# fengranMark/HAConvDR

Hardware: AMD Instinct MI355X
Metric: queries/sec (encode+top-100) over N-passage 768-d corpus; HBM GB/s vs peak (higher is better)
Workload: dtype bf16 MFMA operands with fp32 accumulate / LayerNorm / softmax in the encoder (cosine vs the fp32 reference within 1e-3, measured ~1e-5); search scores and order = the fp32 fmaf chain, bit-exact

## Files before the change

haconvdr_amd/csrc/flat_ip.hip:

```cpp
#include "hac_common.h"

#include <algorithm>
#include <type_traits>
#include <cfloat>
#include <climits>
#include <cmath>
#include <cstdlib>
#include <cstring>
#include <thread>
#include <vector>

namespace hac {

std::string &last_error_slot() {
    static thread_local std::string s;
    return s;
}
int fail(int code, const char *fmt, ...) {
    char buf[512];
    va_list ap;
    va_start(ap, fmt);
    vsnprintf(buf, sizeof buf, fmt, ap);
    va_end(ap);
    last_error_slot() = buf;
// ... 2052 lines not shown
        g.seeded = (size_t)4 * g.GA >= (size_t)SPLIT_K2;
        g.n_pass = scan_passes(G, g.round_groups, g.seeded, g.bounds);
        return g;
    }
    float *delta_of(int64_t off) const { return (float *)ws_delta.p + off; }
    u64 *akeys_of(int64_t off) const { return (u64 *)ws_akeys.p + (size_t)off * SPLIT_K2; }

    int split_begin(SplitCtx &c) {
        const int K2 = SPLIT_K2, C2 = SPLIT_C2;
        const int64_t nq = c.nq;
        hipStream_t st = c.st;
        c.terms = c.level == 0 ? tune.split_terms : 3;
        plan_collect(false);
        HAC_TRY(ensure_half_image(st));
        HAC_TRY(ensure_row_image(st));
        HAC_TRY(upload_segs(st));
        c.G = (u32)((ntotal + GROUP_ROWS - 1) / GROUP_ROWS);
        c.chunk = std::min<int64_t>(nq, SPLIT_CHUNK);
        const int n_qtiles_max = (int)((c.chunk + SH_NQ - 1) / SH_NQ);
        c.lds = c.terms == 3 ? ShCfg<3>::LDS : ShCfg<1>::LDS;
        long Pmax = std::max<long>(1, n_cu);
        HAC_TRY(ws_qsplit.reserve((size_t)n_qtiles_max * SH_NQ * d * 2 * (c.terms == 3 ? 2 : 1)));
        HAC_TRY(ws_delta.reserve((size_t)(nq + SH_NQ) * 4));
        HAC_TRY(ws_cand.reserve((size_t)Pmax * SH_NQ * C2 * 8));
        HAC_TRY(ws_partial.reserve((size_t)std::min<int64_t>(c.chunk, SH_NQ) * Pmax * K2 * 8 * MAX_PASSES));
        HAC_TRY(ws_pcnt.reserve((size_t)c.chunk * 4));
        HAC_TRY(ws_thrglob.reserve(((size_t)n_qtiles_max * SH_NQ + THR_CTL_WORDS) * 4));
        HAC_TRY(ws_akeys.reserve((size_t)nq * K2 * 8));
        HAC_TRY(ws_fail.reserve((size_t)nq * 4));
        HAC_TRY(ws_stat.reserve(16));
        HAC_TRY(ws_thr.reserve((size_t)c.chunk * 4));
        if (((size_t)nq + 8) * 4 > h_fb.cap) HAC_TRY(h_fb.reserve(((size_t)nq + 8) * 8));

        c.a = scan_args(nullptr, 0);
        c.a.pos_base = c.pos_base;
        c.a.k = K2;
        c.a.g_step = 1;
        c.a.thr_glob = thrglob();
        c.a.partial = (u64 *)ws_partial.p;
        c.a.partial_cnt = (u32 *)ws_pcnt.p;
        c.sp.qsplit = (const u32x4 *)ws_qsplit.p;
        c.sp.cand = (u64 *)ws_cand.p;
        c.sp.C2 = C2;
        c.sp.K2 = K2;
        c.sp.thr_is_approx = 1;
        return HAC_OK;
    }
// ... 799 lines not shown
```

haconvdr_amd/csrc/scan_split.inc:

```

typedef _Float16 h16;
typedef _Float16 h16x8 __attribute__((ext_vector_type(8)));
typedef _Float16 h16x4 __attribute__((ext_vector_type(4)));
typedef unsigned int u32x4 __attribute__((ext_vector_type(4)));
typedef float f32x4 __attribute__((ext_vector_type(4)));
typedef const __attribute__((address_space(1))) u32x4 *gu4ptr;

constexpr int SH_NT = 8;
constexpr int SH_NQ = 32 * SH_NT;
constexpr int SH_W = 8;
constexpr int SH_GPR = SH_W / 2;
#ifndef SH_RD1
#define SH_RD1 8
#endif
#ifdef SH_STAMP
#ifndef SH_ST_BX
#define SH_ST_BX 5
#endif
__device__ unsigned long long g_sh_stamps[64];
#endif
template <int TERMS> struct ShCfg {
    static constexpr int STEP_BYTES = TERMS == 3 ? 2048 : 1024;
    static constexpr int CD = TERMS == 3 ? 2 : 1;
    static constexpr int TQ = TERMS == 3 ? 2 : 1;
    static constexpr int STEP_PIECES = SH_NT * TQ * 64;
#ifndef SH_KSL1
#define SH_KSL1 4
#endif
    static constexpr int KSL = TERMS == 3 ? 2 : SH_KSL1;
    static constexpr int SLICE = KSL * STEP_PIECES;
    static constexpr int QS_BYTES = 2 * SLICE * 16;
    static constexpr int RD = TERMS == 3 ? 5 : SH_RD1;
    static constexpr int QDMA = SLICE / (SH_W * 64);
    static constexpr bool SCR_OWN = TERMS == 1;
// ... 56 lines not shown
    for (int o = 32; o > 0; o >>= 1) ss += __shfl_xor(ss, o);
    if ((tid & 63) == 0) red[tid >> 6] = ss;
    __syncthreads();
    if (tid == 0) {
        const int d = 4 * K4;
        const float qn = sqrtf((red[0] + red[1] + red[2]) * 1.0002f);
        const float xn = sqrtf(__uint_as_float(*norm2_max_bits) * 1.0002f);
        float dl = split_err_rel(terms, d) * qn * xn + 1.1920928955078125e-7f * sqrtf((float)d) * (qn + xn) + d * 3.5527136788005009e-15f;
        if (!(qn < 60000.f) || !(xn < 60000.f)) dl = INFINITY;
        delta[qi] = qi < nq ? dl : 0.f;
    }
}

typedef __attribute__((address_space(3))) u32 *lds_u32p;
__device__ __forceinline__ u32 lds_inc_rtn(u32 *p) {
    u32 r;
    const u32 addr = (u32)(uintptr_t)(lds_u32p)p;
    asm volatile("ds_add_rtn_u32 %0, %1, %2\n\ts_waitcnt lgkmcnt(0)" : "=v"(r) : "v"(addr), "v"(1u) : "memory");
    return r;
}
__device__ __forceinline__ void lds_set1(u32 *p) {
    const u32 addr = (u32)(uintptr_t)(lds_u32p)p;
    asm volatile("ds_write_b32 %0, %1" ::"v"(addr), "v"(1u) : "memory");
}

constexpr int q_issues_before(int pos, int rd, int ksl) {
    int c = 0;
    for (int j = 1; j < rd; ++j)
        if ((((pos - j) % ksl) + ksl) % ksl == ksl - 2) ++c;
    return c;
}

template <int N> __device__ __forceinline__ void wait_vmcnt() {
    static_assert(N >= 0 && N < 64, "vmcnt is a 6-bit field");
    __builtin_amdgcn_s_waitcnt(0x0F70 | (N & 15) | ((N >> 4) << 14));
}

#ifndef SH_CORPUS_AUX
#define SH_CORPUS_AUX 0
#endif
#ifndef SH_Q_AUX
#define SH_Q_AUX 0
#endif
template <int TERMS, bool MAXIMA, int QT_ACT = 16>
__global__ __launch_bounds__(SH_W * 64) void scanh_kernel(ScanArgs a, SplitArgs sp) {
    static_assert(QT_ACT == 16 || ((QT_ACT == 8 || QT_ACT == 4) && TERMS == 1), "QT_ACT < 16 is a form of the one-product 16x16x32 scan");
    typedef ShCfg<TERMS> Cfg;
    constexpr int NT = SH_NT, NQ = SH_NQ, W = SH_W, NTHR = SH_W * 64, TQ = Cfg::TQ, RD = Cfg::RD;
    static_assert(Cfg::SCR_OWN || Cfg::SORTERS * 512 * 8 <= Cfg::SLICE * 16, "sort scratch must fit the idle query buffer");
    typedef const __attribute__((address_space(1))) void *gvp;
    typedef __attribute__((address_space(3))) void *lvp;
    extern __shared__ __attribute__((aligned(16))) unsigned char smem[];
    const int tid = threadIdx.x;
    const int lane = tid & 63;
    const int w = __builtin_amdgcn_readfirstlane(tid >> 6);
    const int pr = w >> 1, hf = w & 1;
    const int K4 = a.K4;
    const int NSTEP = K4 / 4;
    const int q0 = blockIdx.y * NQ;
    const int NQr = min(NQ, a.nq - q0);
    const int C2 = sp.C2, K2 = sp.K2;

    u32x4 *qs = reinterpret_cast<u32x4 *>(smem);
    unsigned char *ring = smem + Cfg::QS_BYTES + (size_t)w * RD * Cfg::STEP_BYTES;
    u32 *cnt = reinterpret_cast<u32 *>(smem + Cfg::QS_BYTES + (size_t)W * RD * Cfg::STEP_BYTES);
    float *thr = reinterpret_cast<float *>(cnt + NQ);
    u32 *ovf = reinterpret_cast<u32 *>(thr + NQ);
    u32 *need = ovf + 1;
    SegDesc *lseg = reinterpret_cast<SegDesc *>(ovf + 4);
    u64 *cand = sp.cand + ((size_t)blockIdx.y * gridDim.x + blockIdx.x) * NQ * C2;
    gu4ptr qsrc = (gu4ptr)(sp.qsplit) + (size_t)blockIdx.y * NSTEP * Cfg::STEP_PIECES;

    for (int i = tid; i < NQ; i += NTHR) {
        cnt[i] = 0;
        thr[i] = i < NQr ? (a.thr_init ? a.thr_init[q0 + i] - (sp.thr_is_approx ? 0.f : sp.delta[q0 + i]) : -INFINITY) : __builtin_nanf("");
    }
    if (tid == 0) {
        *ovf = 0;
        *need = 0;
        ovf[2] = 0;
    }
    for (int i = tid; i < Cfg::SLICE; i += NTHR) qs[i] = qsrc[i];
    for (int i = tid; i < a.nseg; i += NTHR) lseg[i] = a.segs[i];
    __syncthreads();
    int seg_cur = 0;
    auto group_base = [&](u32 g) {
        int sg = seg_cur;
        while (sg + 1 < a.nseg && g >= lseg[sg + 1].gstart) ++sg;
        seg_cur = sg;
        if constexpr (TERMS == 3) return as_global(lseg[sg].ptr) + (size_t)(g - lseg[sg].gstart) * K4 * GROUP_ROWS;
        else return as_global(reinterpret_cast<const float4 *>(lseg[sg].himg)) + (size_t)(g - lseg[sg].gstart) * K4 * (GROUP_ROWS / 2);
    };
    const int lane_in_group = TERMS == 3 ? ((lane >> 5) * 64 + 32 * hf + (lane & 31)) : (hf * 64 + lane);
// ... 84 lines not shown
    const int q16_lane = (kg >> 1) * Cfg::STEP_PIECES + (kg & 1) * 32 + m16;

    u32x4 ah, al;
    {
#pragma unroll
        for (int t = 0; t < RD; ++t) dma_step(gp, t, t);
        if constexpr (M16) {
            if (q_issuer) dma_q(1, 1);
        }
        wait_vmcnt<0>();
        __builtin_amdgcn_sched_barrier(0);
        if constexpr (M16) {
#pragma unroll
            for (int rt = 0; rt < 2; ++rt) ac[rt] = *reinterpret_cast<const u32x4 *>(rd16 + rt * 256);
        } else {
            f4 c0, c1;
            read_raw(0, c0, c1);
            convert(c0, c1, ah, al);
        }
        asm volatile("" ::: "memory");
        if constexpr (!LATE) dma_step(gp, RD, 0);
    }
    int rg = 1;
    int par = 0;

#define SH_MFMA(accv, av, bv) \
    accv = __builtin_amdgcn_mfma_f32_32x32x16_f16(__builtin_bit_cast(h16x8, av), __builtin_bit_cast(h16x8, bv), accv, 0, 0, 0)
#define SH_MFMA16(accv, av, bv) \
    accv = __builtin_amdgcn_mfma_f32_16x16x32_f16(__builtin_bit_cast(h16x8, av), __builtin_bit_cast(h16x8, bv), accv, 0, 0, 0)

#ifdef SH_STAMP
    unsigned long long stamps[10] = {0, 0, 0, 0, 0, 0, 0, 0, 0, 0};
#ifdef SH_ST_EPI
#define SH_E(i, rr) if (!MAXIMA && r == (rr)) { \
        const unsigned long long tm_ = __builtin_amdgcn_s_memtime(); \
        const u32 ad_ = (u32)(uintptr_t)(lds_u32p)(smem + Cfg::LDS - 512) + (u32)(w * 64 + (i) * 8); \
        asm volatile("ds_write_b64 %0, %1" ::"v"(ad_), "v"(tm_) : "memory"); }
#else
#define SH_E(i, rr)
#endif
#ifdef SH_ST_ALL
#define SH_T(i) if (((i) == 0 || (i) == 5 || (i) == 8 || (i) == 9) && !MAXIMA && r == SH_ST_R) { \
        const unsigned long long tm_ = __builtin_amdgcn_s_memtime(); \
        const u32 ad_ = (u32)(uintptr_t)(lds_u32p)(smem + Cfg::LDS - 256) + (u32)(w * 32 + ((i) == 0 ? 0 : (i) == 5 ? 8 : (i) == 8 ? 16 : 24)); \
        asm volatile("ds_write_b64 %0, %1" ::"v"(ad_), "v"(tm_) : "memory"); }
#else
#define SH_T(i) if (!MAXIMA && r == SH_ST_R && t >= SH_ST_T && t < SH_ST_T + 4) stamps[i] = __builtin_amdgcn_s_memtime()
#endif
#else
#define SH_E(i, rr)
#define SH_T(i)
#endif
    auto rounds = [&](auto issuer_tag) {
    constexpr int ROLE = decltype(issuer_tag)::value;
    const bool ISSUER = ROLE < 0 ? q_issuer : ROLE == 1;
    for (u32 r = 0; r < nrounds; ++r) {
        const u32 g = a.g_first + item * a.g_step;
        const u32 nitem = item + stride;
        const bool have_next = nitem < a.n_items;
        gf4ptr np = have_next ? uniform(group_base(a.g_first + nitem * a.g_step)) : gp;
        f32x16 acc[NT];
        f32x4 acc16[2][2 * NT];
        if constexpr (!M16) {
#pragma unroll
            for (int n = 0; n < NT; ++n)
#pragma unroll
                for (int e = 0; e < 16; ++e) acc[n][e] = 0.f;
        }

        auto step = [&](const int t, auto pos_tag) {
            constexpr int POS = decltype(pos_tag)::value;
            if constexpr (M16) {
                const u32x4 *qb_cur = qs + par * Cfg::SLICE + q16_lane, *qb_nxt = qs + (par ^ 1) * Cfg::SLICE + q16_lane;
                auto bfrag = [&](int buf, int pp, int qt) {
                    return (buf == par ? qb_cur : qb_nxt)[2 * pp * Cfg::STEP_PIECES + (qt >> 1) * 64 + (qt & 1) * 16];
                };
                constexpr int PP = POS >> 1, ODD = POS & 1;
                constexpr bool LASTP = POS == Cfg::KSL - 1;
                SH_T(POS * 2 + 0);
                if (POS == 0 && t == 0) { SH_E(4, SH_ST_R + 1); }
                if (POS == 1 && t == 1) { SH_E(6, SH_ST_R + 1); }
                asm volatile("" ::: "memory");
                if (POS == 0 && t == 0) {
#pragma unroll
                    for (int i = 0; i < BD; ++i)
                        if (i < QT_ACT) bq[i][0] = bfrag(par, 0, i);
                }
                auto tiles = [&](auto fresh_tag) {
                    constexpr bool FRESH = decltype(fresh_tag)::value;
#pragma unroll
                    for (int i = 0; i < 8; ++i) {
                        const int qt = ODD * 8 + i;
                        const u32x4 bh = bq[i][0];
                        if (qt < QT_ACT) {
                        if constexpr (FRESH) {
                            const f32x4 zero = {0.f, 0.f, 0.f, 0.f};
                            acc16[0][qt] = __builtin_amdgcn_mfma_f32_16x16x32_f16(__builtin_bit_cast(h16x8, ac[0]), __builtin_bit_cast(h16x8, bh), zero, 0, 0, 0);
                            acc16[1][qt] = __builtin_amdgcn_mfma_f32_16x16x32_f16(__builtin_bit_cast(h16x8, ac[1]), __builtin_bit_cast(h16x8, bh), zero, 0, 0, 0);
                        } else {
                            SH_MFMA16(acc16[0][qt], ac[0], bh);
                            SH_MFMA16(acc16[1][qt], ac[1], bh);
                        }
                        }
                        if (!ODD) {
                            if (8 + i < QT_ACT) bq[i][0] = bfrag(par, PP, 8 + i);
                        } else if (i < QT_ACT) {
                            if (!LASTP) bq[i][0] = bfrag(par, PP + 1, i);
                            else if (t + 1 < NSTEP) bq[i][0] = bfrag(par ^ 1, 0, i);
                        }
                        __builtin_amdgcn_sched_barrier(0);
                    }
                };
                if (POS < 2 && t == POS) tiles(std::true_type{});
                else tiles(std::false_type{});
                asm volatile("" ::: "memory");
                SH_T(POS * 2 + 1);
                if (POS == 0 && t == 0) { SH_E(5, SH_ST_R + 1); }
                auto handover = [&]() {
                    asm volatile("" ::: "memory");
                    if (ISSUER) wait_vmcnt<Cfg::CD * Cfg::KSL>();
                    asm volatile("s_waitcnt lgkmcnt(0)" ::: "memory");
                    SH_T(8);
                    __builtin_amdgcn_s_barrier();
                    SH_T(9);
                    __builtin_amdgcn_sched_barrier(0);
                    const int NSL = NSTEP / Cfg::KSL;
                    int sn = t / Cfg::KSL + 2;
                    if (sn >= NSL) sn -= NSL;
                    if (ISSUER) dma_q(sn, par);
                };
                if (ODD) {
                    constexpr int LA = LATE ? 1 : 0;
                    constexpr int QISS = q_issues_before(POS, RD - LA, Cfg::KSL);
                    if constexpr (QFAST) {
                        if (ISSUER) wait_vmcnt<Cfg::CD * (RD - 2 - LA) + QISS * 2 * Cfg::QDMA>();
                        else wait_vmcnt<Cfg::CD * (RD - 2 - LA)>();
                    } else {
                        wait_vmcnt<Cfg::CD * (RD - 2 - LA) + QISS * Cfg::QDMA>();
                    }
                    __builtin_amdgcn_sched_barrier(0);
#pragma unroll
                    for (int rt = 0; rt < 2; ++rt) ac[rt] = *reinterpret_cast<const u32x4 *>(rd16 + rg * 1024 + rt * 256);
                    if constexpr (!LATE) asm volatile("s_waitcnt lgkmcnt(0)" ::: "memory");
                }
                if constexpr (LATE) {
                    const int tn = t + RD, rs = rg == 0 ? RD - 1 : rg - 1;
                    if (tn < NSTEP) dma_step(gp, tn, rs);
                    else dma_step(np, tn - NSTEP, rs);
                    rg = rg == RD - 1 ? 0 : rg + 1;
                } else {
                    const int tn = t + RD + 1;
                    if (tn < NSTEP) dma_step(gp, tn, rg);
                    else dma_step(np, tn - NSTEP, rg);
                    rg = rg == RD - 1 ? 0 : rg + 1;
                }
                if (POS == Cfg::KSL - 2) handover();
                if (LASTP) par ^= 1;
                __builtin_amdgcn_sched_barrier(0);
                return;
            }
            constexpr int OPENERS = POS == 0 ? RD / Cfg::KSL : (POS <= RD ? (RD - POS) / Cfg::KSL + 1 : 0);
            asm volatile("" ::: "memory");
            wait_vmcnt<Cfg::CD * (RD - 1) + OPENERS * Cfg::QDMA>();
            __builtin_amdgcn_sched_barrier(0);
            u32x4 nh, nl;
            const u32x4 *qcur = qs + par * Cfg::SLICE + POS * Cfg::STEP_PIECES + lane;
            if (POS == 0) {
#pragma unroll
                for (int i = 0; i < BD; ++i)
#pragma unroll
                    for (int h = 0; h < TQ; ++h) bq[i][h] = qcur[(i * TQ + h) * 64];
            }
            f4 c0, c1;
            read_raw(rg, c0, c1);
#pragma unroll
            for (int n = 0; n < NT; ++n) {
                const u32x4 bh = bq[n % BD][0];
                if (TERMS == 3) {
                    const u32x4 bl = bq[n % BD][TQ - 1];
// ... 13 lines not shown
            }
            asm volatile("" ::: "memory");
            {
                const int tn = t + RD + 1;
                if (tn < NSTEP) dma_step(gp, tn, rg);
                else dma_step(np, tn - NSTEP, rg);
                rg = rg == RD - 1 ? 0 : rg + 1;
            }
            if (POS == 0) {
                asm volatile("" ::: "memory");
                __builtin_amdgcn_sched_barrier(0);
                const int sn = t / Cfg::KSL + 1;
                dma_q(sn == NSTEP / Cfg::KSL ? 0 : sn, par ^ 1);
            }
            if (POS == Cfg::KSL - 1) {
                wait_vmcnt<Cfg::CD * (Cfg::KSL - 1)>();
                __builtin_amdgcn_s_barrier();
                par ^= 1;
            }
            ah = nh;
            al = nl;
            __builtin_amdgcn_sched_barrier(0);
        };
        for (int t = 0; t < NSTEP; t += Cfg::KSL) {
            step(t, std::integral_constant<int, 0>{});
            step(t + 1, std::integral_constant<int, 1>{});
            if constexpr (Cfg::KSL >= 4) {
                step(t + 2, std::integral_constant<int, 2>{});
                step(t + 3, std::integral_constant<int, 3>{});
            }
            if constexpr (Cfg::KSL == 8) {
                step(t + 4, std::integral_constant<int, 4>{});
                step(t + 5, std::integral_constant<int, 5>{});
                step(t + 6, std::integral_constant<int, 6>{});
                step(t + 7, std::integral_constant<int, 7>{});
            }
        }
        SH_E(0, SH_ST_R);
        gp = np;
        if constexpr (MAXIMA) {
            if (have) {
                const long rem = a.n_rows - (long)g * GROUP_ROWS;
                const int rows_valid = rem < GROUP_ROWS ? (int)rem : GROUP_ROWS;
                const int rb = 32 * hf + 4 * hh;
                const size_t S = (size_t)4 * a.n_items;
                if constexpr (M16) {
#pragma unroll
                    for (int qt = 0; qt < (QT_ACT < 2 * NT ? QT_ACT : 2 * NT); ++qt)
#pragma unroll
                        for (int rt = 0; rt < 2; ++rt) {
                            float m = -INFINITY;
#pragma unroll
                            for (int e = 0; e < 4; ++e)
                                if (32 * hf + 16 * rt + 4 * kg + e < rows_valid) m = fmaxf(m, acc16[rt][qt][e]);
                            m = fmaxf(m, __shfl_xor(m, 16));
                            m = fmaxf(m, __shfl_xor(m, 32));
                            if (kg == 0 && qt * 16 + m16 < NQr) sp.maxima[(size_t)(q0 + qt * 16 + m16) * S + (size_t)item * 4 + hf * 2 + rt] = m;
                        }
                } else {
#pragma unroll
                for (int n = 0; n < NT; ++n) {
                    float m = -INFINITY;
#pragma unroll
                    for (int e = 0; e < 16; ++e)
                        if ((e & 3) + 8 * (e >> 2) + rb < rows_valid) m = fmaxf(m, acc[n][e]);
                    if (n * 32 + jl < NQr) sp.maxima[(size_t)(q0 + n * 32 + jl) * S + (size_t)item * 4 + hf * 2 + hh] = m;
                }
                }
            }
            item = nitem;
            have = have_next;
            continue;
        }
#if SH_NOEPI == 1
#pragma unroll
        for (int rt = 0; rt < 2; ++rt)
            asm volatile("" ::"v"(acc16[rt][0]), "v"(acc16[rt][1]), "v"(acc16[rt][2]), "v"(acc16[rt][3]), "v"(acc16[rt][4]), "v"(acc16[rt][5]), "v"(acc16[rt][6]), "v"(acc16[rt][7]),
                         "v"(acc16[rt][8]), "v"(acc16[rt][9]), "v"(acc16[rt][10]), "v"(acc16[rt][11]), "v"(acc16[rt][12]), "v"(acc16[rt][13]), "v"(acc16[rt][14]), "v"(acc16[rt][15]));
        item = nitem;
        have = have_next;
        continue;
#endif
        constexpr bool STAGED = M16 && Cfg::SCR_OWN;
        constexpr int REGION = Cfg::SORTERS * 4096 / SH_W;
#ifdef SH_REC_CAP
        constexpr int REC_CAP = SH_REC_CAP;
#else
        constexpr int REC_CAP = REGION / 48 < 64 ? REGION / 48 : 64;
#endif
        static_assert(!STAGED || (REGION % 16 == 0 && REC_CAP * 48 <= REGION && REC_CAP <= 64), "staging region");
        unsigned char *stg = smem + Cfg::LDS_BASE + (size_t)w * REGION;
        const u32 stg_a = (u32)(uintptr_t)(lds_u32p)stg;
        f32x4 rec0 = {0.f, 0.f, 0.f, 0.f}, rec1 = {0.f, 0.f, 0.f, 0.f};
        u32 rcode = 0u, rfull = 0u;
        u64 *scr = reinterpret_cast<u64 *>(Cfg::SCR_OWN ? smem + Cfg::LDS_BASE : smem + (size_t)(par ^ 1) * Cfg::SLICE * 16) + (size_t)(w % Cfg::SORTERS) * C2;

        constexpr int NTL = M16 ? (QT_ACT < 2 * NT ? QT_ACT : 2 * NT) : NT, NE = M16 ? 8 : 16;
        constexpr int PB = 32 / NE, PMASK = (1 << NE) - 1;
        u32 pw[NTL / PB];
#pragma unroll
        for (int i = 0; i < NTL / PB; ++i) pw[i] = 0u;
        auto pget = [&](int n) { return (pw[n / PB] >> ((n % PB) * NE)) & (u32)PMASK; };
        const int rbase = 32 * hf + 4 * hh;
        auto qof = [&](int tl) { return M16 ? tl * 16 + m16 : tl * 32 + jl; };
        u32 qlc = (u32)(M16 ? m16 : jl) * (u32)C2;
        asm volatile("" : "+v"(qlc));
        auto rof = [&](int x) { return M16 ? 32 * hf + 16 * (x >> 2) + 4 * kg + (x & 3) : (x & 3) + 8 * (x >> 2) + rbase; };
        auto vof = [&](int tl, int x) -> float {
            if constexpr (M16) return acc16[x >> 2][tl][x & 3];
            else return acc[tl][x];
        };
        auto append_record = [&](u32 m) -> u32 {
            const int pl = (int)(rcode & 63u), pn = (int)(rcode >> 8);
            const int pj = pn * 16 + (pl & 15);
            u32 full = 0u;
            while (__any(m != 0u)) {
                if (m != 0u) {
                    const int e = __builtin_ctz(m);
                    m &= m - 1u;
                    float sc = rec0[0];
#pragma unroll
                    for (int x = 1; x < 8; ++x) sc = e == x ? (x < 4 ? rec0[x & 3] : rec1[x & 3]) : sc;
                    const u32 pos = lds_inc_rtn(&cnt[pj]);
                    if (pos < (u32)C2) {
                        const int row = 32 * hf + 16 * (e >> 2) + 4 * (pl >> 4) + (e & 3);
                        cand[(u32)pj * (u32)C2 + pos] = make_key(sc, a.pos_base + g * GROUP_ROWS + row);
                        if (pos >= hw) lds_set1(need);
                    } else {
                        lds_set1(ovf);
                        full |= 1u << e;
                    }
                }
            }
            return full;
        };
        bool direct = false;
        {
            const long rem = a.n_rows - (long)g * GROUP_ROWS;
            const int rows_valid = rem < GROUP_ROWS ? (int)rem : GROUP_ROWS;
            float thn[NTL];
#pragma unroll
            for (int n = 0; n < NTL; ++n) thn[n] = thr[qof(n)];
            asm volatile("s_waitcnt lgkmcnt(0)" ::: "memory");
            if constexpr (STAGED) {
                int base = 0;
                if (have) {
#pragma unroll
                    for (int n = 0; n < NTL; ++n) {
                        const float th = thn[n];
                        float mx;
                        asm("v_max3_f32 %0, %1, %2, %3" : "=v"(mx) : "v"(vof(n, 0)), "v"(vof(n, 1)), "v"(vof(n, 2)));
                        asm("v_max3_f32 %0, %1, %2, %3" : "=v"(mx) : "v"(mx), "v"(vof(n, 3)), "v"(vof(n, 4)));
                        asm("v_max3_f32 %0, %1, %2, %3" : "=v"(mx) : "v"(mx), "v"(vof(n, 5)), "v"(vof(n, 6)));
                        asm("v_max_f32 %0, %1, %2" : "=v"(mx) : "v"(mx), "v"(vof(n, 7)));
                        const unsigned long long bal = __ballot(mx >= th);
                        const int nf = __builtin_popcountll(bal);
                        if (nf == 0) continue;
                        if (base + nf > REC_CAP) {
                            direct = true;
#pragma unroll
                            for (int e = 0; e < NE; ++e) {
                                if (vof(n, e) >= th && rof(e) < rows_valid) pw[n / PB] |= (1u << (e + (n % PB) * NE));
                            }
                        } else {
                            const u32 rank = __builtin_amdgcn_mbcnt_hi((u32)(bal >> 32), __builtin_amdgcn_mbcnt_lo((u32)bal, 0u));
                            const u32 ad = stg_a + __umul24((u32)base + rank, 48u);
                            const u32 code = (u32)(n << 8) | (u32)lane;
                            unsigned long long sv;
                            asm volatile("s_and_saveexec_b64 %0, %1\n\tds_write_b128 %2, %3\n\tds_write_b128 %2, %4 offset:16\n\t"
                                         "ds_write2_b32 %2, %5, %6 offset0:8 offset1:9\n\ts_mov_b64 exec, %0"
                                         : "=&s"(sv)
                                         : "s"(bal), "v"(ad), "v"(acc16[0][n]), "v"(acc16[1][n]), "v"(code), "v"(th)
                                         : "memory", "scc");
                            base += nf;
                        }
                    }
                }
                if (base > 0) {
                    u32 m = 0u;
                    if (lane < base) {
                        const unsigned char *rp = stg + lane * 48;
                        rec0 = *reinterpret_cast<const f32x4 *>(rp);
                        rec1 = *reinterpret_cast<const f32x4 *>(rp + 16);
                        rcode = *reinterpret_cast<const u32 *>(rp + 32);
                        const float rth = *reinterpret_cast<const float *>(rp + 36);
#pragma unroll
                        for (int e = 0; e < 4; ++e) {
                            m |= rec0[e] >= rth ? (1u << e) : 0u;
                            m |= rec1[e] >= rth ? (16u << e) : 0u;
                        }
                        if (rows_valid != GROUP_ROWS) {
#pragma unroll
                            for (int e = 0; e < 8; ++e)
                                if (32 * hf + 16 * (e >> 2) + 4 * (int)((rcode & 63u) >> 4) + (e & 3) >= rows_valid) m &= ~(1u << e);
                        }
                    }
                    rfull = append_record(m);
                }
            } else {
#pragma unroll
            for (int n = 0; n < NTL; ++n) {
                const float th = thn[n];
                if (have) {
                    float mx;
                    if constexpr (NE == 8) {
                        asm("v_max3_f32 %0, %1, %2, %3" : "=v"(mx) : "v"(vof(n, 0)), "v"(vof(n, 1)), "v"(vof(n, 2)));
                        asm("v_max3_f32 %0, %1, %2, %3" : "=v"(mx) : "v"(mx), "v"(vof(n, 3)), "v"(vof(n, 4)));
                        asm("v_max3_f32 %0, %1, %2, %3" : "=v"(mx) : "v"(mx), "v"(vof(n, 5)), "v"(vof(n, 6)));
                        asm("v_max_f32 %0, %1, %2" : "=v"(mx) : "v"(mx), "v"(vof(n, 7)));
                    } else {
                        mx = vof(n, 0);
#pragma unroll
                        for (int e = 1; e < NE; ++e) mx = fmaxf(mx, vof(n, e));
                    }
#if SH_NOEPI == 3
                    asm volatile("" ::"v"(mx));
                    if (false) {
#else
                    if (__any(mx >= th)) {
#endif
#pragma unroll
                        for (int e = 0; e < NE; ++e) {
// ... 1 lines not shown
                            if (v >= th && (rows_valid == GROUP_ROWS || rof(e) < rows_valid)) {
#if SH_NOEPI == 2
                                asm volatile("" ::"v"(v));
                                continue;
#endif
                                const u32 pos = lds_inc_rtn(&cnt[qof(n)]);
                                if (pos < (u32)C2) {
                                    cand[(u32)(n * (M16 ? 16 : 32) * C2) + qlc + pos] = make_key(v, a.pos_base + g * GROUP_ROWS + rof(e));
                                    if (pos >= hw) lds_set1(need);
                                } else {
                                    lds_set1(ovf);
                                    pw[n / PB] |= (1u << (e + (n % PB) * NE));
                                }
                            }
                        }
                    }
                }
            }
            }
        }
        SH_E(1, SH_ST_R);
        for (int pass = 0;; ++pass) {
            bool anyp = false;
            if (pass > 0 || direct) {
#pragma unroll
                for (int i = 0; i < NTL / PB; ++i) anyp |= (pw[i] != 0u);
            }
            if ((pass > 0 || direct) && __any(anyp)) {
#pragma unroll
                for (int n = 0; n < NTL; ++n) {
                    if (pget(n) != 0u) {
                        float sc[NE];
#pragma unroll
                        for (int e = 0; e < NE; ++e) sc[e] = vof(n, e);
                        const int j = qof(n);
                        u32 m = pget(n);
                        while (m) {
                            const int e = __builtin_ctz(m);
                            m &= m - 1u;
                            const u32 pos = lds_inc_rtn(&cnt[j]);
                            if (pos < (u32)C2) {
                                const int row = rof(e);
                                cand[(u32)(n * (M16 ? 16 : 32) * C2) + qlc + pos] = make_key(sc[e], a.pos_base + g * GROUP_ROWS + row);
                                pw[n / PB] &= ~(1u << (e + (n % PB) * NE));
                                if (pos >= hw) lds_set1(need);
                            } else {
                                lds_set1(ovf);
                            }
                        }
                    }
                }
            }
            if constexpr (STAGED) {
                if (pass > 0 && __any(rfull != 0u)) rfull = append_record(rfull);
            }
            if (pass == 0) {
                SH_E(2, SH_ST_R);
                __builtin_amdgcn_s_waitcnt(0xC07F);
                __builtin_amdgcn_s_barrier();
                SH_E(3, SH_ST_R);
                if ((*(volatile u32 *)ovf | *(volatile u32 *)need) == 0u) break;
            }
            __syncthreads();
            const bool over = (*ovf != 0u);
            for (int jj = w; jj < NQr && w < Cfg::SORTERS; jj += Cfg::SORTERS) {
                u32 n = cnt[jj];
                if (n > (u32)C2) n = (u32)C2;
                float t_new = -INFINITY;
                const bool compact = n > hw;
                if (compact) {
                    u64 *cj = cand + (size_t)jj * C2;
                    for (u32 i = lane; i < n; i += 64) scr[i] = cj[i];
                    lds_fence();
                    wave_sort_desc(scr, n, lane);
                    t_new = ord2f((u32)(scr[K2 - 1] >> 32));
                    for (u32 i = lane; i < (u32)K2; i += 64) cj[i] = scr[i];
                }
                if (lane == 0) {
// ... 5 lines not shown
                            atomicMax(&a.thr_glob[q0 + jj], f2ord(t_new));
                        }
                    }
                    const u32 go = __hip_atomic_load(&a.thr_glob[q0 + jj], __ATOMIC_RELAXED, __HIP_MEMORY_SCOPE_AGENT);
                    if (go != 0u) t_cur = fmaxf(t_cur, ord2f(go));
                    thr[jj] = t_cur;
                }
            }
            __syncthreads();
            if (tid == 0) {
                *ovf = 0u;
                *need = 0u;
                ovf[2] = over ? ovf[2] + 1u : 0u;
            }
            if (!over) break;
#pragma unroll
            for (int n = 0; n < NTL; ++n) {
                if (pget(n) == 0u) continue;
                const float th = thr[qof(n)];
#pragma unroll
                for (int e = 0; e < NE; ++e)
                    if ((pw[n / PB] & (1u << (e + (n % PB) * NE))) && !(vof(n, e) >= th)) pw[n / PB] &= ~(1u << (e + (n % PB) * NE));
            }
            if constexpr (STAGED) {
                if (rfull != 0u) {
                    const float th = thr[(int)(rcode >> 8) * 16 + (int)(rcode & 15u)];
#pragma unroll
                    for (int e = 0; e < 8; ++e)
                        if ((rfull & (1u << e)) && !((e < 4 ? rec0[e & 3] : rec1[e & 3]) >= th)) rfull &= ~(1u << e);
                }
            }
            __syncthreads();
            if (__builtin_expect(*(volatile u32 *)(ovf + 2) >= scan_pass_bound(a, SH_GPR * 64 + 4), 0)) {
                static_assert(NQ <= NTHR, "one thread per query of the tile");
                scan_overrun(a, q0, NQr, tid);
                __syncthreads();
                if (tid == 0) ovf[2] = 0u;
                break;
            }
        }
        item = nitem;
        have = have_next;
    }
    };
    if constexpr (QFAST && !MAXIMA) {
        if (w < 4) rounds(std::integral_constant<int, 1>{});
        else rounds(std::integral_constant<int, 0>{});
    } else if constexpr (QFAST) {
        rounds(std::integral_constant<int, -1>{});
    } else {
        rounds(std::integral_constant<int, 1>{});
    }
#undef SH_MFMA

    wait_vmcnt<0>();
#ifdef SH_STAMP
    if (!MAXIMA) {
        __syncthreads();
        for (int i = tid; i < NQ; i += NTHR) atomicAdd(&g_sh_stamps[60], (unsigned long long)min(cnt[i], (u32)C2));
    }
    if (!MAXIMA && blockIdx.x == SH_ST_BX && blockIdx.y == 0 && lane == 0) {
#ifdef SH_ST_EPI
        for (int i = 0; i < 7; ++i) g_sh_stamps[w * 8 + i] = reinterpret_cast<const unsigned long long *>(smem + Cfg::LDS - 512)[w * 8 + i];
#elif defined(SH_ST_ALL)
        for (int i = 0; i < 4; ++i) g_sh_stamps[w * 4 + i] = reinterpret_cast<const unsigned long long *>(smem + Cfg::LDS - 256)[w * 4 + i];
// ... 254 lines not shown
```

Baseline: 8268.

## Weave previous group's threshold filtering into next group's MFMA steps

In the M16 staged path, the per-group epilogue (max-reduce, ballot, staging survivors to LDS, appending candidates) is deferred and interleaved with the next group's MFMA tiles. The previous group's accumulators are kept live, filtered tile by tile during the first steps, and survivors that overflow the LDS staging area are parked in a new per-wave global spill region appended to the candidate workspace. The goal is to hide the epilogue's latency and barrier behind matrix work. In exchange it adds register pressure from the duplicated accumulators, extra global spill traffic, and considerably more complex control flow.

```diff
diff --git a/haconvdr_amd/csrc/flat_ip.hip b/haconvdr_amd/csrc/flat_ip.hip
--- a/haconvdr_amd/csrc/flat_ip.hip
+++ b/haconvdr_amd/csrc/flat_ip.hip
@@ -2098,7 +2098,7 @@
         long Pmax = std::max<long>(1, n_cu);
         HAC_TRY(ws_qsplit.reserve((size_t)n_qtiles_max * SH_NQ * d * 2 * (c.terms == 3 ? 2 : 1)));
         HAC_TRY(ws_delta.reserve((size_t)(nq + SH_NQ) * 4));
-        HAC_TRY(ws_cand.reserve((size_t)Pmax * SH_NQ * C2 * 8));
+        HAC_TRY(ws_cand.reserve((size_t)Pmax * ((size_t)SH_NQ * C2 + SH_SPILL_U64) * 8));
         HAC_TRY(ws_partial.reserve((size_t)std::min<int64_t>(c.chunk, SH_NQ) * Pmax * K2 * 8 * MAX_PASSES));
         HAC_TRY(ws_pcnt.reserve((size_t)c.chunk * 4));
         HAC_TRY(ws_thrglob.reserve(((size_t)n_qtiles_max * SH_NQ + THR_CTL_WORDS) * 4));
diff --git a/haconvdr_amd/csrc/scan_split.inc b/haconvdr_amd/csrc/scan_split.inc
--- a/haconvdr_amd/csrc/scan_split.inc
+++ b/haconvdr_amd/csrc/scan_split.inc
@@ -10,6 +10,9 @@
 constexpr int SH_NQ = 32 * SH_NT;
 constexpr int SH_W = 8;
 constexpr int SH_GPR = SH_W / 2;
+constexpr int SH_SPILL_REC = 2 * SH_NT * 64;
+constexpr size_t SH_SPILL_U64 = (size_t)SH_W * SH_SPILL_REC * 6;
+constexpr u32 SH_REC_FRESH = 0x80000000u;
 #ifndef SH_RD1
 #define SH_RD1 8
 #endif
@@ -112,6 +115,10 @@
 __device__ __forceinline__ void lds_set1(u32 *p) {
     const u32 addr = (u32)(uintptr_t)(lds_u32p)p;
     asm volatile("ds_write_b32 %0, %1" ::"v"(addr), "v"(1u) : "memory");
+}
+__device__ __forceinline__ void lds_set1_w(u32 *p) {
+    const u32 addr = (u32)(uintptr_t)(lds_u32p)p;
+    asm volatile("ds_write_b32 %0, %1\n\ts_waitcnt lgkmcnt(0)" ::"v"(addr), "v"(1u) : "memory");
 }
 
 constexpr int q_issues_before(int pos, int rd, int ksl) {
@@ -158,7 +165,7 @@
     u32 *ovf = reinterpret_cast<u32 *>(thr + NQ);
     u32 *need = ovf + 1;
     SegDesc *lseg = reinterpret_cast<SegDesc *>(ovf + 4);
-    u64 *cand = sp.cand + ((size_t)blockIdx.y * gridDim.x + blockIdx.x) * NQ * C2;
+    u64 *cand = sp.cand + ((size_t)blockIdx.y * gridDim.x + blockIdx.x) * ((size_t)NQ * C2 + SH_SPILL_U64);
     gu4ptr qsrc = (gu4ptr)(sp.qsplit) + (size_t)blockIdx.y * NSTEP * Cfg::STEP_PIECES;
 
     for (int i = tid; i < NQ; i += NTHR) {
@@ -289,6 +296,9 @@
         if constexpr (!LATE) dma_step(gp, RD, 0);
     }
     int rg = 1;
+    u32 fp_g = 0;
+    bool fp_have = false;
+    int brec = 0;
     int par = 0;
 
 #define SH_MFMA(accv, av, bv) \
@@ -321,13 +331,230 @@
     auto rounds = [&](auto issuer_tag) {
     constexpr int ROLE = decltype(issuer_tag)::value;
     const bool ISSUER = ROLE < 0 ? q_issuer : ROLE == 1;
+    constexpr bool WEAVE = M16 && Cfg::SCR_OWN && !MAXIMA && SH_NOEPI != 1;
+    constexpr int NTL16 = QT_ACT < 2 * NT ? QT_ACT : 2 * NT;
+    constexpr int WREGION = Cfg::SORTERS * 4096 / SH_W;
+#ifdef SH_REC_CAP
+    constexpr int WREC_CAP = SH_REC_CAP;
+#else
+    constexpr int WREC_CAP = WREGION / 48 < 64 ? WREGION / 48 : 64;
+#endif
+    static_assert(!WEAVE || (WREGION % 16 == 0 && WREC_CAP * 48 <= WREGION && WREC_CAP <= 64 && Cfg::KSL >= 4), "staging region; filter steps before the first hand-over");
+    f32x4 acc16_w[2][2 * NT];
+    auto fp_rows_valid = [&](const u32 fg) __attribute__((always_inline)) {
+        const long rem = a.n_rows - (long)fg * GROUP_ROWS;
+        return rem < GROUP_ROWS ? (int)rem : GROUP_ROWS;
+    };
+    auto spill_of = [&]() __attribute__((always_inline)) { return reinterpret_cast<u32x4 *>(cand + (size_t)NQ * C2) + (size_t)w * SH_SPILL_REC * 3; };
+    auto append_rec = [&](u32 m, const f32x4 &r0, const f32x4 &r1, const u32 code, const u32 fg) __attribute__((always_inline)) -> u32 {
+        const int pl = (int)(code & 63u), pn = (int)(code >> 8);
+        const int pj = pn * 16 + (pl & 15);
+        u32 full = 0u;
+        while (__any(m != 0u)) {
+            if (m != 0u) {
+                const int e = __builtin_ctz(m);
+                m &= m - 1u;
+                float sc = r0[0];
+#pragma unroll
+                for (int x = 1; x < 8; ++x) sc = e == x ? (x < 4 ? r0[x & 3] : r1[x & 3]) : sc;
+                const u32 pos = lds_inc_rtn(&cnt[pj]);
+                if (pos < (u32)C2) {
+                    const int row = 32 * hf + 16 * (e >> 2) + 4 * (pl >> 4) + (e & 3);
+                    cand[(u32)pj * (u32)C2 + pos] = make_key(sc, a.pos_base + fg * GROUP_ROWS + row);
+                    if (pos >= hw) lds_set1_w(need);
+                } else {
+                    lds_set1_w(ovf);
+                    full |= 1u << e;
+                }
+            }
+        }
+        return full;
+    };
+    auto park = [&, spill_of](const int n, const float th, const unsigned long long bal, const int st, const u32 fg) __attribute__((always_inline)) -> int {
+        const int nrec = st & 255, ngl = st >> 8;
+        const int nf = __builtin_popcountll(bal);
+        const u32 rank = __builtin_amdgcn_mbcnt_hi((u32)(bal >> 32), __builtin_amdgcn_mbcnt_lo((u32)bal, 0u));
+        u32 ln = (u32)lane;
+        asm volatile("" : "+v"(ln));
+        const u32 code = (u32)(n << 8) | ln;
+        if (nrec + nf <= WREC_CAP) {
+            const u32 ad = (u32)(uintptr_t)(lds_u32p)(smem + Cfg::LDS_BASE + (size_t)w * WREGION) + __umul24((u32)nrec + rank, 48u);
+            unsigned long long sv;
+            asm volatile("s_and_saveexec_b64 %0, %1\n\tds_write_b128 %2, %3\n\tds_write_b128 %2, %4 offset:16\n\t"
+                         "ds_write2_b32 %2, %5, %6 offset0:8 offset1:9\n\ts_mov_b64 exec, %0\n\ts_waitcnt lgkmcnt(0)"
+                         : "=&s"(sv)
+                         : "s"(bal), "v"(ad), "v"(acc16_w[0][n]), "v"(acc16_w[1][n]), "v"(code), "v"(th)
+                         : "memory", "scc");
+            return st + nf;
+        } else {
+            if ((bal >> ln) & 1ull) {
+                u32x4 *rp = spill_of() + (size_t)((u32)ngl + rank) * 3;
+                rp[0] = __builtin_bit_cast(u32x4, acc16_w[0][n]);
+                rp[1] = __builtin_bit_cast(u32x4, acc16_w[1][n]);
+                const u32x4 c = {code, __float_as_uint(th), SH_REC_FRESH, 0u};
+                rp[2] = c;
+            }
+            return st + 256 * nf;
+        }
+    };
+    auto filt_tile = [&, park](const int n, const float th, const int st, const u32 fg) __attribute__((always_inline)) -> int {
+        float mx;
+        asm("v_max3_f32 %0, %1, %2, %3" : "=v"(mx) : "v"(acc16_w[0][n][0]), "v"(acc16_w[0][n][1]), "v"(acc16_w[0][n][2]));
+        asm("v_max3_f32 %0, %1, %2, %3" : "=v"(mx) : "v"(mx), "v"(acc16_w[0][n][3]), "v"(acc16_w[1][n][0]));
+        asm("v_max3_f32 %0, %1, %2, %3" : "=v"(mx) : "v"(mx), "v"(acc16_w[1][n][1]), "v"(acc16_w[1][n][2]));
+        asm("v_max_f32 %0, %1, %2" : "=v"(mx) : "v"(mx), "v"(acc16_w[1][n][3]));
+        const unsigned long long bal = __ballot(mx >= th);
+        if (bal != 0ull) return park(n, th, bal, st, fg);
+        return st;
+    };
+    auto records = [&, append_rec, spill_of, fp_rows_valid](const bool retry, const int st, const u32 fg) __attribute__((always_inline)) -> int {
+        u32x4 *spill = spill_of();
+        const int nrec = st & 255, ngl0 = st >> 8;
+        int ngl = ngl0;
+        if (ngl0 > 0) __builtin_amdgcn_fence(__ATOMIC_SEQ_CST, "workgroup");
+        for (int b0 = 0; b0 < ngl0; b0 += 64) {
+            const int i = b0 + lane;
+            u32 m = 0u, om = 0u, code = 0u;
+            f32x4 r0 = {0.f, 0.f, 0.f, 0.f}, r1 = {0.f, 0.f, 0.f, 0.f};
+            if (i < ngl0) {
+                const u32x4 c = spill[(size_t)i * 3 + 2];
+                om = m = c[2];
+                if (m != 0u) {
+                    r0 = __builtin_bit_cast(f32x4, spill[(size_t)i * 3]);
+                    r1 = __builtin_bit_cast(f32x4, spill[(size_t)i * 3 + 1]);
+                    code = c[0];
+                    if (m == SH_REC_FRESH) {
+                        const float rth = __uint_as_float(c[1]);
+                        m = 0u;
+#pragma unroll
+                        for (int e = 0; e < 4; ++e) {
+                            m |= r0[e] >= rth ? (1u << e) : 0u;
+                            m |= r1[e] >= rth ? (16u << e) : 0u;
+                        }
+                        const int rows_valid = fp_rows_valid(fg);
+                        if (rows_valid != GROUP_ROWS) {
+#pragma unroll
+                            for (int e = 0; e < 8; ++e)
+                                if (32 * hf + 16 * (e >> 2) + 4 * (int)((code & 63u) >> 4) + (e & 3) >= rows_valid) m &= ~(1u << e);
+                        }
+                    }
+                    if (retry) {
+                        const float th = thr[(int)(code >> 8) * 16 + (int)(code & 15u)];
+#pragma unroll
+                        for (int e = 0; e < 8; ++e)
+                            if (!((e < 4 ? r0[e & 3] : r1[e & 3]) >= th)) m &= ~(1u << e);
+                    }
+                }
+            }
+            if (!__any(om != 0u)) continue;
+            const u32 full = append_rec(m, r0, r1, code, fg);
+            if (om != full) reinterpret_cast<u32 *>(spill + (size_t)i * 3 + 2)[2] = full;
+        }
+        if (!retry && nrec > 0) {
+            u32 m = 0u, code = 0u;
+            float rth = 0.f;
+            f32x4 r0 = {0.f, 0.f, 0.f, 0.f}, r1 = {0.f, 0.f, 0.f, 0.f};
+            if (lane < nrec) {
+                const unsigned char *rp = smem + Cfg::LDS_BASE + (size_t)w * WREGION + lane * 48;
+                r0 = *reinterpret_cast<const f32x4 *>(rp);
+                r1 = *reinterpret_cast<const f32x4 *>(rp + 16);
+                code = *reinterpret_cast<const u32 *>(rp + 32);
+                rth = *reinterpret_cast<const float *>(rp + 36);
+#pragma unroll
+                for (int e = 0; e < 4; ++e) {
+                    m |= r0[e] >= rth ? (1u << e) : 0u;
+                    m |= r1[e] >= rth ? (16u << e) : 0u;
+                }
+                const int rows_valid = fp_rows_valid(fg);
+                if (rows_valid != GROUP_ROWS) {
+#pragma unroll
+                    for (int e = 0; e < 8; ++e)
+                        if (32 * hf + 16 * (e >> 2) + 4 * (int)((code & 63u) >> 4) + (e & 3) >= rows_valid) m &= ~(1u << e);
+                }
+            }
+            const u32 full = append_rec(m, r0, r1, code, fg);
+            const unsigned long long fb = __ballot(full != 0u);
+            if (fb != 0ull) {
+                const u32 rank = __builtin_amdgcn_mbcnt_hi((u32)(fb >> 32), __builtin_amdgcn_mbcnt_lo((u32)fb, 0u));
+                if (full != 0u) {
+                    u32x4 *rp = spill + (size_t)((u32)ngl + rank) * 3;
+                    rp[0] = __builtin_bit_cast(u32x4, r0);
+                    rp[1] = __builtin_bit_cast(u32x4, r1);
+                    const u32x4 c = {code, __float_as_uint(rth), full, 0u};
+                    rp[2] = c;
+                }
+                ngl += __builtin_popcountll(fb);
+            }
+        }
+        return 256 * ngl;
+    };
+    auto compact_lists = [&, records](int st, const u32 fg) __attribute__((always_inline)) {
+        u64 *scr = reinterpret_cast<u64 *>(smem + Cfg::LDS_BASE) + (size_t)(w % Cfg::SORTERS) * C2;
+        for (;;) {
+            __syncthreads();
+            const bool over = (*ovf != 0u);
+            for (int jj = w; jj < NQr && w < Cfg::SORTERS; jj += Cfg::SORTERS) {
+                u32 n = cnt[jj];
+                if (n > (u32)C2) n = (u32)C2;
+                float t_new = -INFINITY;
+                const bool compact = n > hw;
+                if (compact) {
+                    u64 *cj = cand + (size_t)jj * C2;
+                    for (u32 i = lane; i < n; i += 64) scr[i] = cj[i];
+                    lds_fence();
+                    wave_sort_desc(scr, n, lane);
+                    t_new = ord2f((u32)(scr[K2 - 1] >> 32));
+                    for (u32 i = lane; i < (u32)K2; i += 64) cj[i] = scr[i];
+                }
+                if (lane == 0) {
+                    float t_cur = thr[jj];
+                    if (compact) {
+                        cnt[jj] = K2;
+                        if (t_new > t_cur) {
+                            t_cur = t_new;
+                            atomicMax(&a.thr_glob[q0 + jj], f2ord(t_new));
+                        }
+                    }
+                    const u32 go = __hip_atomic_load(&a.thr_glob[q0 + jj], __ATOMIC_RELAXED, __HIP_MEMORY_SCOPE_AGENT);
+                    if (go != 0u) t_cur = fmaxf(t_cur, ord2f(go));
+                    thr[jj] = t_cur;
+                }
+            }
+            __syncthreads();
+            if (tid == 0) {
+                *ovf = 0u;
+                *need = 0u;
+                ovf[2] = over ? ovf[2] + 1u : 0u;
+            }
+            if (!over) break;
+            __syncthreads();
+            if (__builtin_expect(*(volatile u32 *)(ovf + 2) >= scan_pass_bound(a, SH_GPR * 64 + 4), 0)) {
+                static_assert(NQ <= NTHR, "one thread per query of the tile");
+                scan_overrun(a, q0, NQr, tid);
+                __syncthreads();
+                if (tid == 0) ovf[2] = 0u;
+                break;
+            }
+            st = records(true, st, fg);
+        }
+    };
+    if constexpr (WEAVE) {
+#pragma unroll
+        for (int rt = 0; rt < 2; ++rt)
+#pragma unroll
+            for (int qt = 0; qt < 2 * NT; ++qt) acc16_w[rt][qt] = f32x4{0.f, 0.f, 0.f, 0.f};
+#pragma unroll
+        for (int i = 0; i < BD; ++i)
+            if (i < QT_ACT) bq[i][0] = (qs + par * Cfg::SLICE + q16_lane)[(i >> 1) * 64 + (i & 1) * 16];
+    }
     for (u32 r = 0; r < nrounds; ++r) {
         const u32 g = a.g_first + item * a.g_step;
         const u32 nitem = item + stride;
         const bool have_next = nitem < a.n_items;
-        gf4ptr np = have_next ? uniform(group_base(a.g_first + nitem * a.g_step)) : gp;
+        gf4ptr np = !WEAVE && have_next ? uniform(group_base(a.g_first + nitem * a.g_step)) : gp;
         f32x16 acc[NT];
-        f32x4 acc16[2][2 * NT];
+        f32x4 acc16_r[2][2 * NT];
+        auto &acc16 = *(WEAVE ? &acc16_w : &acc16_r);
         if constexpr (!M16) {
 #pragma unroll
             for (int n = 0; n < NT; ++n)
@@ -335,8 +562,10 @@
                 for (int e = 0; e < 16; ++e) acc[n][e] = 0.f;
         }
 
-        auto step = [&](const int t, auto pos_tag) {
+        auto step = [&, filt_tile, records, compact_lists](const int t, auto pos_tag, auto first_tag) {
             constexpr int POS = decltype(pos_tag)::value;
+            constexpr bool FIRST = decltype(first_tag)::value;
+            (void)filt_tile, (void)records, (void)compact_lists;
             if constexpr (M16) {
                 const u32x4 *qb_cur = qs + par * Cfg::SLICE + q16_lane, *qb_nxt = qs + (par ^ 1) * Cfg::SLICE + q16_lane;
                 auto bfrag = [&](int buf, int pp, int qt) {
@@ -348,18 +577,28 @@
                 if (POS == 0 && t == 0) { SH_E(4, SH_ST_R + 1); }
                 if (POS == 1 && t == 1) { SH_E(6, SH_ST_R + 1); }
                 asm volatile("" ::: "memory");
-                if (POS == 0 && t == 0) {
+                if (FIRST && POS == 0 && !WEAVE) {
 #pragma unroll
                     for (int i = 0; i < BD; ++i)
                         if (i < QT_ACT) bq[i][0] = bfrag(par, 0, i);
                 }
-                auto tiles = [&](auto fresh_tag) {
-                    constexpr bool FRESH = decltype(fresh_tag)::value;
+                auto tiles = [&, filt_tile](auto fresh_tag, auto filt_tag) {
+                    constexpr bool FRESH = decltype(fresh_tag)::value, FILT = decltype(filt_tag)::value;
+                    float thc = 0.f;
+                    if constexpr (FILT) {
+                        if (ODD * 8 < QT_ACT) thc = thr[ODD * 8 * 16 + m16];
+                    }
 #pragma unroll
                     for (int i = 0; i < 8; ++i) {
                         const int qt = ODD * 8 + i;
                         const u32x4 bh = bq[i][0];
                         if (qt < QT_ACT) {
+                        if constexpr (FILT) {
+                            float thn = 0.f;
+                            if (i + 1 < 8 && qt + 1 < QT_ACT) thn = thr[(qt + 1) * 16 + m16];
+                            brec = filt_tile(qt, fp_have ? thc : __builtin_nanf(""), brec, fp_g);
+                            thc = thn;
+                        }
                         if constexpr (FRESH) {
                             const f32x4 zero = {0.f, 0.f, 0.f, 0.f};
                             acc16[0][qt] = __builtin_amdgcn_mfma_f32_16x16x32_f16(__builtin_bit_cast(h16x8, ac[0]), __builtin_bit_cast(h16x8, bh), zero, 0, 0, 0);
@@ -373,13 +612,21 @@
                             if (8 + i < QT_ACT) bq[i][0] = bfrag(par, PP, 8 + i);
                         } else if (i < QT_ACT) {
                             if (!LASTP) bq[i][0] = bfrag(par, PP + 1, i);
-                            else if (t + 1 < NSTEP) bq[i][0] = bfrag(par ^ 1, 0, i);
+                            else if (WEAVE || t + 1 < NSTEP) bq[i][0] = bfrag(par ^ 1, 0, i);
                         }
                         __builtin_amdgcn_sched_barrier(0);
                     }
                 };
-                if (POS < 2 && t == POS) tiles(std::true_type{});
-                else tiles(std::false_type{});
+                u32 flags = 0u;
+                if constexpr (WEAVE && FIRST && LASTP) flags = *(volatile u32 *)ovf | *(volatile u32 *)need;
+                if constexpr (FIRST && POS < 2) {
+                    tiles(std::true_type{}, std::integral_constant<bool, WEAVE>{});
+                    if constexpr (WEAVE && POS == 1) {
+                        if (brec != 0) brec = records(false, brec, fp_g);
+                    }
+                } else {
+                    tiles(std::false_type{}, std::false_type{});
+                }
                 asm volatile("" ::: "memory");
                 SH_T(POS * 2 + 1);
                 if (POS == 0 && t == 0) { SH_E(5, SH_ST_R + 1); }
@@ -422,6 +669,16 @@
                     rg = rg == RD - 1 ? 0 : rg + 1;
                 }
                 if (POS == Cfg::KSL - 2) handover();
+                if constexpr (WEAVE && FIRST && LASTP) {
+                    if (flags != 0u) {
+                        compact_lists(brec, fp_g);
+#pragma unroll
+                        for (int i = 0; i < BD; ++i)
+                            if (i < QT_ACT) bq[i][0] = bfrag(par ^ 1, 0, i);
+                    }
+                    brec = 0;
+                    if (have_next) np = uniform(group_base(a.g_first + nitem * a.g_step));
+                }
                 if (LASTP) par ^= 1;
                 __builtin_amdgcn_sched_barrier(0);
                 return;
@@ -481,19 +738,25 @@
             al = nl;
             __builtin_amdgcn_sched_barrier(0);
         };
-        for (int t = 0; t < NSTEP; t += Cfg::KSL) {
-            step(t, std::integral_constant<int, 0>{});
-            step(t + 1, std::integral_constant<int, 1>{});
+        auto slice = [&](const int t, auto first_tag) {
+            step(t, std::integral_constant<int, 0>{}, first_tag);
+            step(t + 1, std::integral_constant<int, 1>{}, first_tag);
             if constexpr (Cfg::KSL >= 4) {
-                step(t + 2, std::integral_constant<int, 2>{});
-                step(t + 3, std::integral_constant<int, 3>{});
+                step(t + 2, std::integral_constant<int, 2>{}, first_tag);
+                step(t + 3, std::integral_constant<int, 3>{}, first_tag);
             }
             if constexpr (Cfg::KSL == 8) {
-                step(t + 4, std::integral_constant<int, 4>{});
-                step(t + 5, std::integral_constant<int, 5>{});
-                step(t + 6, std::integral_constant<int, 6>{});
-                step(t + 7, std::integral_constant<int, 7>{});
-            }
+                step(t + 4, std::integral_constant<int, 4>{}, first_tag);
+                step(t + 5, std::integral_constant<int, 5>{}, first_tag);
+                step(t + 6, std::integral_constant<int, 6>{}, first_tag);
+                step(t + 7, std::integral_constant<int, 7>{}, first_tag);
+            }
+        };
+        if constexpr (M16) {
+            slice(0, std::true_type{});
+            for (int t = Cfg::KSL; t < NSTEP; t += Cfg::KSL) slice(t, std::false_type{});
+        } else {
+            for (int t = 0; t < NSTEP; t += Cfg::KSL) slice(t, std::false_type{});
         }
         SH_E(0, SH_ST_R);
         gp = np;
@@ -531,6 +794,13 @@
             have = have_next;
             continue;
         }
+        if constexpr (WEAVE) {
+            fp_g = g;
+            fp_have = have;
+            item = nitem;
+            have = have_next;
+            continue;
+        }
 #if SH_NOEPI == 1
 #pragma unroll
         for (int rt = 0; rt < 2; ++rt)
@@ -540,18 +810,6 @@
         have = have_next;
         continue;
 #endif
-        constexpr bool STAGED = M16 && Cfg::SCR_OWN;
-        constexpr int REGION = Cfg::SORTERS * 4096 / SH_W;
-#ifdef SH_REC_CAP
-        constexpr int REC_CAP = SH_REC_CAP;
-#else
-        constexpr int REC_CAP = REGION / 48 < 64 ? REGION / 48 : 64;
-#endif
-        static_assert(!STAGED || (REGION % 16 == 0 && REC_CAP * 48 <= REGION && REC_CAP <= 64), "staging region");
-        unsigned char *stg = smem + Cfg::LDS_BASE + (size_t)w * REGION;
-        const u32 stg_a = (u32)(uintptr_t)(lds_u32p)stg;
-        f32x4 rec0 = {0.f, 0.f, 0.f, 0.f}, rec1 = {0.f, 0.f, 0.f, 0.f};
-        u32 rcode = 0u, rfull = 0u;
         u64 *scr = reinterpret_cast<u64 *>(Cfg::SCR_OWN ? smem + Cfg::LDS_BASE : smem + (size_t)(par ^ 1) * Cfg::SLICE * 16) + (size_t)(w % Cfg::SORTERS) * C2;
 
         constexpr int NTL = M16 ? (QT_ACT < 2 * NT ? QT_ACT : 2 * NT) : NT, NE = M16 ? 8 : 16;
@@ -569,31 +827,6 @@
             if constexpr (M16) return acc16[x >> 2][tl][x & 3];
             else return acc[tl][x];
         };
-        auto append_record = [&](u32 m) -> u32 {
-            const int pl = (int)(rcode & 63u), pn = (int)(rcode >> 8);
-            const int pj = pn * 16 + (pl & 15);
-            u32 full = 0u;
-            while (__any(m != 0u)) {
-                if (m != 0u) {
-                    const int e = __builtin_ctz(m);
-                    m &= m - 1u;
-                    float sc = rec0[0];
-#pragma unroll
-                    for (int x = 1; x < 8; ++x) sc = e == x ? (x < 4 ? rec0[x & 3] : rec1[x & 3]) : sc;
-                    const u32 pos = lds_inc_rtn(&cnt[pj]);
-                    if (pos < (u32)C2) {
-                        const int row = 32 * hf + 16 * (e >> 2) + 4 * (pl >> 4) + (e & 3);
-                        cand[(u32)pj * (u32)C2 + pos] = make_key(sc, a.pos_base + g * GROUP_ROWS + row);
-                        if (pos >= hw) lds_set1(need);
-                    } else {
-                        lds_set1(ovf);
-                        full |= 1u << e;
-                    }
-                }
-            }
-            return full;
-        };
-        bool direct = false;
         {
             const long rem = a.n_rows - (long)g * GROUP_ROWS;
             const int rows_valid = rem < GROUP_ROWS ? (int)rem : GROUP_ROWS;
@@ -601,62 +834,7 @@
 #pragma unroll
             for (int n = 0; n < NTL; ++n) thn[n] = thr[qof(n)];
             asm volatile("s_waitcnt lgkmcnt(0)" ::: "memory");
-            if constexpr (STAGED) {
-                int base = 0;
-                if (have) {
-#pragma unroll
-                    for (int n = 0; n < NTL; ++n) {
-                        const float th = thn[n];
-                        float mx;
-                        asm("v_max3_f32 %0, %1, %2, %3" : "=v"(mx) : "v"(vof(n, 0)), "v"(vof(n, 1)), "v"(vof(n, 2)));
-                        asm("v_max3_f32 %0, %1, %2, %3" : "=v"(mx) : "v"(mx), "v"(vof(n, 3)), "v"(vof(n, 4)));
-                        asm("v_max3_f32 %0, %1, %2, %3" : "=v"(mx) : "v"(mx), "v"(vof(n, 5)), "v"(vof(n, 6)));
-                        asm("v_max_f32 %0, %1, %2" : "=v"(mx) : "v"(mx), "v"(vof(n, 7)));
-                        const unsigned long long bal = __ballot(mx >= th);
-                        const int nf = __builtin_popcountll(bal);
-                        if (nf == 0) continue;
-                        if (base + nf > REC_CAP) {
-                            direct = true;
-#pragma unroll
-                            for (int e = 0; e < NE; ++e) {
-                                if (vof(n, e) >= th && rof(e) < rows_valid) pw[n / PB] |= (1u << (e + (n % PB) * NE));
-                            }
-                        } else {
-                            const u32 rank = __builtin_amdgcn_mbcnt_hi((u32)(bal >> 32), __builtin_amdgcn_mbcnt_lo((u32)bal, 0u));
-                            const u32 ad = stg_a + __umul24((u32)base + rank, 48u);
-                            const u32 code = (u32)(n << 8) | (u32)lane;
-                            unsigned long long sv;
-                            asm volatile("s_and_saveexec_b64 %0, %1\n\tds_write_b128 %2, %3\n\tds_write_b128 %2, %4 offset:16\n\t"
-                                         "ds_write2_b32 %2, %5, %6 offset0:8 offset1:9\n\ts_mov_b64 exec, %0"
-                                         : "=&s"(sv)
-                                         : "s"(bal), "v"(ad), "v"(acc16[0][n]), "v"(acc16[1][n]), "v"(code), "v"(th)
-                                         : "memory", "scc");
-                            base += nf;
-                        }
-                    }
-                }
-                if (base > 0) {
-                    u32 m = 0u;
-                    if (lane < base) {
-                        const unsigned char *rp = stg + lane * 48;
-                        rec0 = *reinterpret_cast<const f32x4 *>(rp);
-                        rec1 = *reinterpret_cast<const f32x4 *>(rp + 16);
-                        rcode = *reinterpret_cast<const u32 *>(rp + 32);
-                        const float rth = *reinterpret_cast<const float *>(rp + 36);
-#pragma unroll
-                        for (int e = 0; e < 4; ++e) {
-                            m |= rec0[e] >= rth ? (1u << e) : 0u;
-                            m |= rec1[e] >= rth ? (16u << e) : 0u;
-                        }
-                        if (rows_valid != GROUP_ROWS) {
-#pragma unroll
-                            for (int e = 0; e < 8; ++e)
-                                if (32 * hf + 16 * (e >> 2) + 4 * (int)((rcode & 63u) >> 4) + (e & 3) >= rows_valid) m &= ~(1u << e);
-                        }
-                    }
-                    rfull = append_record(m);
-                }
-            } else {
+            {
 #pragma unroll
             for (int n = 0; n < NTL; ++n) {
                 const float th = thn[n];
@@ -704,11 +882,11 @@
         SH_E(1, SH_ST_R);
         for (int pass = 0;; ++pass) {
             bool anyp = false;
-            if (pass > 0 || direct) {
+            if (pass > 0) {
 #pragma unroll
                 for (int i = 0; i < NTL / PB; ++i) anyp |= (pw[i] != 0u);
             }
-            if ((pass > 0 || direct) && __any(anyp)) {
+            if (pass > 0 && __any(anyp)) {
 #pragma unroll
                 for (int n = 0; n < NTL; ++n) {
                     if (pget(n) != 0u) {
@@ -733,9 +911,6 @@
                     }
                 }
             }
-            if constexpr (STAGED) {
-                if (pass > 0 && __any(rfull != 0u)) rfull = append_record(rfull);
-            }
             if (pass == 0) {
                 SH_E(2, SH_ST_R);
                 __builtin_amdgcn_s_waitcnt(0xC07F);
@@ -787,14 +962,6 @@
                 for (int e = 0; e < NE; ++e)
                     if ((pw[n / PB] & (1u << (e + (n % PB) * NE))) && !(vof(n, e) >= th)) pw[n / PB] &= ~(1u << (e + (n % PB) * NE));
             }
-            if constexpr (STAGED) {
-                if (rfull != 0u) {
-                    const float th = thr[(int)(rcode >> 8) * 16 + (int)(rcode & 15u)];
-#pragma unroll
-                    for (int e = 0; e < 8; ++e)
-                        if ((rfull & (1u << e)) && !((e < 4 ? rec0[e & 3] : rec1[e & 3]) >= th)) rfull &= ~(1u << e);
-                }
-            }
             __syncthreads();
             if (__builtin_expect(*(volatile u32 *)(ovf + 2) >= scan_pass_bound(a, SH_GPR * 64 + 4), 0)) {
                 static_assert(NQ <= NTHR, "one thread per query of the tile");
@@ -806,6 +973,20 @@
         }
         item = nitem;
         have = have_next;
+    }
+    if constexpr (WEAVE) {
+        if (fp_have) {
+            float thn[NTL16];
+#pragma unroll
+            for (int n = 0; n < NTL16; ++n) thn[n] = thr[n * 16 + m16];
+#pragma unroll
+            for (int n = 0; n < NTL16; ++n) brec = filt_tile(n, thn[n], brec, fp_g);
+        }
+        if (brec != 0) brec = records(false, brec, fp_g);
+        wait_vmcnt<0>();
+        __builtin_amdgcn_s_waitcnt(0xC07F);
+        __builtin_amdgcn_s_barrier();
+        if ((*(volatile u32 *)ovf | *(volatile u32 *)need) != 0u) compact_lists(brec, fp_g);
     }
     };
     if constexpr (QFAST && !MAXIMA) {
```

New measurement: 8311 (median of 6 runs). Within noise of the previous version (+0.5%).
